# WujiangXu/AMID

Hardware: AMD Instinct MI355X
Metric: train samples/sec (higher is better)
Workload: dtype f32; 1 GPU; cloth_sport_train75-shaped SASRec train step (BASELINE.json configs[1]); batch_per_gpu=256, global_batch=256, seq_len=50, emb_dim=128, hid_dim=32, neg=1, table_rows=894820, unique_rows_last_step=1921, input=HBM-resident batch pool, dropout=on (p=0.5), optimizer=Adam (dense-equivalent lazy rows), graph=True, steps_per_graph=1, parallelism=dp1

## Files before the change

### amid_amd/csrc/adam.hip

```cpp
#include "common.h"
#include "rng.h"
#include "sort_phases.h"
#include "adam_replay.h"
#include "live_list.h"
#include "seg_spans.h"
#include "tail_parts.h"
#include "reduce_partials.h"
#include "weights_image.h"
#include "pool_slab.h"

namespace amid {

template <int MODE>
__global__ __launch_bounds__(256) void lazy_adam_rows_kernel(float* __restrict__ table, float* __restrict__ m_tab, float* __restrict__ v_tab,
                                                             int* __restrict__ last, const int* __restrict__ uniq_ids,
                                                             const int* __restrict__ n_uniq_p, const float* __restrict__ uniq_grad, int D,
                                                             const StepState* __restrict__ stp, float grad_scale) {
    __shared__ IdleCoef tab[COEF_TAB];
    const StepState st = *stp;
    const int U = *n_uniq_p;
    const int sub = threadIdx.x & 31;
    const int hw0 = blockIdx.x * (blockDim.x >> 5) + (threadIdx.x >> 5), n_hw = gridDim.x * (blockDim.x >> 5);
    if (blockIdx.x * (blockDim.x >> 5) >= U) return;
    fill_coef_table(tab, st);
// ... 356 lines not shown
        st4(g + i, gg);
        return gg;
    }
    __device__ __forceinline__ float one(long long k) const {
        float gs = reduced ? g[k] : d0[k];
        for (int r = 1; !reduced && r < world; ++r) gs += d0[r * chunk_floats + k];
        g[k] = gs;
        return gs;
    }
};

__global__ __launch_bounds__(256) void optimizer_gathered_kernel(float* __restrict__ p, float* __restrict__ m, float* __restrict__ v,
                                                                 float* __restrict__ g, long long n, int dense_blocks,
                                                                 float* __restrict__ table, float* __restrict__ m_tab, float* __restrict__ v_tab,
                                                                 int* __restrict__ last, const float* __restrict__ gathered, int world, int umax,
                                                                 long long chunk_floats, int id_rows, long long dense_off, int D, int sentinel,
                                                                 const StepState* __restrict__ stp, float grad_scale) {
    __shared__ IdleCoef tab[COEF_TAB];
    const StepState st = *stp;
    if ((int)blockIdx.x < dense_blocks) {
        dense_adam_range(p, m, v, n, blockIdx.x, dense_blocks, GatheredDenseGrad{g, gathered + dense_off, dense_off < 0, world, chunk_floats}, grad_scale,
                         adam_coef_now(st));
        return;
    }
    const int rb = blockIdx.x - dense_blocks, n_rb = gridDim.x - dense_blocks;
    const int total = world * umax;
    if (rb * 8 >= total) return;
    fill_coef_table(tab, st);
    const AdamCoef cnow = adam_coef_now(st);
    const int sub = threadIdx.x & 31;
    for (int u = rb * 8 + (threadIdx.x >> 5); u < total; u += n_rb * 8) {
        const int r0 = u / umax, i0 = u - r0 * umax;
        const int x = ((const int*)(gathered + r0 * chunk_floats))[i0];
        if (x >= sentinel) continue;
        const int half = (threadIdx.x >> 5) & 1;
        int j = -1;
        if (sub < world && sub != r0) j = find_id((const int*)(gathered + sub * chunk_floats), umax, x);
        const unsigned int fm = (unsigned int)(__ballot(j >= 0) >> (32 * half));
        if (fm & ((1u << r0) - 1u)) continue;
        const auto grad = [&](int c) {
            float4 gg = ld4(gathered + r0 * chunk_floats + (long long)(id_rows + i0) * D + 4 * c);
            for (int r = r0 + 1; r < world; ++r) {
                const int jr = __shfl(j, 32 * half + r);
                if ((fm >> r) & 1u) {
                    const float4 tt = ld4(gathered + r * chunk_floats + (long long)(id_rows + jr) * D + 4 * c);
                    gg.x += tt.x; gg.y += tt.y; gg.z += tt.z; gg.w += tt.w;
                }
            }
            return gg;
        };
        halfwave_row<ROW_STEP>(table, m_tab, v_tab, last, x, D, sub, st, tab, cnow, grad_scale, grad);
    }
}


struct DenseAdamSink {
    float* p; float* m; float* v; const float* g0; long long n; AdamCoef c; float gs;
    __device__ __forceinline__ void quad(float* dst, float4 g) const {
        const long long off = dst - g0;
        if (off < 0 || off + 4 > n) return;
        dense_quad_step(p, m, v, off, g, gs, c);
    }
    __device__ __forceinline__ void one(float* dst, float g) const {
        const long long off = dst - g0;
        if (off < 0 || off >= n) return;
        dense_elem_step(p, m, v, off, g, gs, c);
    }
};

struct DenseShipSink {
    const float* g0; long long n; float* dst;
    __device__ __forceinline__ void quad(float* d, float4 g) const {
        const long long off = d - g0;
        if (dst == nullptr || off < 0 || off + 4 > n) return;
        st4(dst + off, g);
    }
    __device__ __forceinline__ void one(float* d, float g) const {
        const long long off = d - g0;
        if (dst == nullptr || off < 0 || off >= n) return;
        dst[off] = g;
    }
};

struct TailOptArgs {
    const float* grad_rows; const int* pos_sorted; const int* seg_off; const int* seg_of; int n_sorted;
    float* uniq_grad; float* partial; int n_seg, nch; int* ticket;
    const ReduceEntry* entries; const int* blk_off; int n_entries, n_red;
    PosSum ps;
    float* p; float* m; float* v; float* g; long long n_dense; long long left_lo, left_hi; int left_blocks;
    float* table; float* m_tab; float* v_tab; int* last; const int* uniq_ids; const int* n_uniq; int row_blocks;
    const StepState* st; float grad_scale;
    float* dense_dst; int* out_ids; int n_out, pad_id, id_blocks; int* err;
};

template <int VEC, bool APPLY>
__global__ __launch_bounds__(256) void grad_tail_opt_kernel(const TailOptArgs a) {
    constexpr int D = VEC * 64;
    __shared__ IdleCoef tab[COEF_TAB];
    StepState st = {};
    if constexpr (APPLY) st = *a.st;
    const long long t = st.step;
    int bid = blockIdx.x;
    if (bid < a.n_seg) {
        segreduce_chunks_block<VEC, true>(a.grad_rows, a.pos_sorted, a.seg_of, a.n_sorted, nullptr, a.partial, bid, SEG_CHUNK, a.seg_off);
        asm volatile("s_waitcnt vmcnt(0)" ::: "memory");
        __shared__ int s_last, s_n;
        __shared__ int owners[256];
        __shared__ float red[16][D];
        __syncthreads();
        if (threadIdx.x == 0) s_last = (atomicAdd(a.ticket, 1) == a.n_seg - 1) ? 1 : 0;
        __syncthreads();
        if (!s_last) return;
        if (threadIdx.x == 0) *a.ticket = 0;
        AdamCoef cnow = {};
        if constexpr (APPLY) cnow = adam_coef_now(st);
        bool tab_filled = false;
        for (int c0 = 0; c0 < a.nch; c0 += 256) {
            if (threadIdx.x == 0) s_n = 0;
            __syncthreads();
            {
                const int c = c0 + (int)threadIdx.x;
                int u, cl;
                if (c < a.nch && spans_owner(c, a.seg_off, a.seg_of, a.n_sorted, SEG_CHUNK, u, cl) && a.seg_off[u + 1] - a.seg_off[u] > SEG_CHUNK)
                    owners[atomicAdd(&s_n, 1)] = c;
            }
            __syncthreads();
            const int n_own = s_n;
            for (int k = 0; k < n_own; ++k) {
                const int c = owners[k];
                int u = 0, c_last = 0;
                spans_owner(c, a.seg_off, a.seg_of, a.n_sorted, SEG_CHUNK, u, c_last);
                long long r = 0, l = 0;
                if constexpr (APPLY) { r = a.uniq_ids[u]; l = a.last[r]; }
                const bool lag = APPLY && row_owes(l, catchup_end(t));
                const int cq0 = threadIdx.x;
                float4 pp0 = make_float4(0.f, 0.f, 0.f, 0.f), mm0 = pp0, vv0 = pp0;
                if constexpr (APPLY) {
                    if (cq0 < D / 4) { const long long off = r * D + 4 * cq0; pp0 = ld4(a.table + off); mm0 = ld4(a.m_tab + off); vv0 = ld4(a.v_tab + off); }
                }
                spans_partials<VEC, 4, true>(red, c, c_last, a.partial);
                if (lag && !tab_filled) { fill_coef_table(tab, st); tab_filled = true; }
                __syncthreads();
                for (int cq = threadIdx.x; cq < D / 4; cq += blockDim.x) {
                    const float4 gs = make_float4(spans_total<VEC>(red, 4 * cq), spans_total<VEC>(red, 4 * cq + 1), spans_total<VEC>(red, 4 * cq + 2),
                                                  spans_total<VEC>(red, 4 * cq + 3));
                    st4(a.uniq_grad + (long long)u * D + 4 * cq, gs);
                    if constexpr (APPLY) {
                        const long long off = r * D + 4 * cq;
                        float4 pp = pp0, mm = mm0, vv = vv0;
                        row_quad_step(pp, mm, vv, gs, a.grad_scale, l, lag, st, tab, cnow);
                        st4(a.table + off, pp); st4(a.m_tab + off, mm); st4(a.v_tab + off, vv);
                    }
                }
                if constexpr (APPLY) { if (threadIdx.x == 0) a.last[r] = (int)t; }
                __syncthreads();
            }
        }
        return;
    }
    bid -= a.n_seg;
    auto make_sink = [&]() {
        if constexpr (APPLY) {
            DenseAdamSink k;
            k.p = a.p; k.m = a.m; k.v = a.v; k.g0 = a.g; k.n = a.n_dense; k.c = adam_coef_now(st); k.gs = a.grad_scale;
            return k;
        } else {
            return DenseShipSink{a.g, a.n_dense, a.dense_dst};
        }
    };
    const auto sink = make_sink();
    if (bid < a.n_red) {
        int lo = 0, hi = a.n_entries;
        while (hi - lo > 1) {
            const int mid = (lo + hi) >> 1;
            if (a.blk_off[mid] <= bid) lo = mid; else hi = mid;
        }
        reduce_partials_block(a.entries[lo], bid - a.blk_off[lo], a.blk_off[lo + 1] - a.blk_off[lo], sink);
        return;
    }
    bid -= a.n_red;
    if (bid < 2 * a.ps.nblk) {
        pos_sum_block(a.ps, D, bid / a.ps.nblk, bid % a.ps.nblk, a.ps.nblk, sink);
        return;
    }
    bid -= 2 * a.ps.nblk;
    if (bid < a.left_blocks) {
        for (long long i = a.left_lo + ((long long)bid * blockDim.x + threadIdx.x) * 4; i < a.left_hi; i += (long long)a.left_blocks * blockDim.x * 4) {
            if (i + 4 <= a.left_hi) sink.quad(a.g + i, ld4(a.g + i));
            else for (long long k = i; k < a.left_hi; ++k) sink.one(a.g + k, a.g[k]);
        }
        return;
    }
    bid -= a.left_blocks;
    if constexpr (!APPLY) {
        if (bid < a.id_blocks) {
            const int rr = bid * 256 + (int)threadIdx.x;
            if (rr < a.n_out) a.out_ids[rr] = rr < *a.n_uniq ? a.uniq_ids[rr] : a.pad_id;
            if (rr == 0 && a.err != nullptr && *a.n_uniq > a.n_out) atomicOr(a.err, AMID_FLAG_UMAX_EXCEEDED);
            return;
        }
        bid -= a.id_blocks;
    }
    {
        const int U = *a.n_uniq;
        if (bid * 8 >= U) return;
        AdamCoef cnow = {};
        if constexpr (APPLY) { fill_coef_table(tab, st); cnow = adam_coef_now(st); }
        const int sub = threadIdx.x & 31;
        for (int u = bid * 8 + (threadIdx.x >> 5); u < U; u += a.row_blocks * 8) {
            const int s0 = a.seg_off[u], s1 = a.seg_off[u + 1];
            if (s1 - s0 > SEG_CHUNK) continue;
            const int mid = min(s1, (s0 / SEG_CHUNK + 1) * SEG_CHUNK);
            const auto grad = [&](int c) {
                auto piece = [&](int e, const int e_end) {
                    float4 acc = make_float4(0.f, 0.f, 0.f, 0.f);
                    for (; e + 8 <= e_end; e += 8) {
                        int ps_[8];
#pragma unroll
                        for (int j = 0; j < 8; ++j) ps_[j] = a.pos_sorted[e + j];
                        float4 rw[8];
#pragma unroll
                        for (int j = 0; j < 8; ++j) rw[j] = ld4(a.grad_rows + (long long)ps_[j] * D + 4 * c);
#pragma unroll
                        for (int j = 0; j < 8; ++j) acc = f4add(acc, rw[j]);
                    }
                    for (; e < e_end; ++e) acc = f4add(acc, ld4(a.grad_rows + (long long)a.pos_sorted[e] * D + 4 * c));
                    return acc;
                };
                float4 gs = piece(s0, mid);
                if (mid < s1) {
                    const float4 z = make_float4(0.f, 0.f, 0.f, 0.f);
                    const float4 r0 = f4add(z, gs), r1 = f4add(z, piece(mid, s1));
                    gs = f4add(f4add(z, r0), r1);
                }
                st4(a.uniq_grad + (long long)u * D + 4 * c, gs);
                return gs;
            };
            halfwave_row<APPLY ? ROW_STEP : ROW_SHIP>(a.table, a.m_tab, a.v_tab, a.last, APPLY ? a.uniq_ids[u] : 0, D, sub, st, tab, cnow, a.grad_scale, grad);
        }
        return;
    }
}

}

using namespace amid;

extern "C" int amid_step_state_bytes(void) { return (int)sizeof(StepState); }

extern "C" int amid_step_state_pack(void* host_buf, unsigned long long seed, long long step, double lr, double beta1, double beta2, double eps) {
    AMID_CHECK_ARG(host_buf);
    StepState s;
    s.seed = seed; s.step = step; s.lr = lr; s.beta1 = beta1; s.beta2 = beta2; s.eps = eps; s.ticket = 0; s.pad_ = 0; s.step_done = step;
    *(StepState*)host_buf = s;
    return AMID_OK;
}

extern "C" int amid_step_begin(void* step_state, void* stream) {
    AMID_CHECK_ARG(step_state);
    step_begin_kernel<<<1, 1, 0, (hipStream_t)stream>>>((StepState*)step_state);
    AMID_LAUNCH_CHECK();
    return AMID_OK;
}

static inline int dense_grid(long long n, int cap) {
    long long b = (n / 4 + 255) / 256;
    if (b < 1) b = 1;
    if (b > cap) b = cap;
    return (int)b;
}

static inline int rows_grid(long long n_rows_hint) {
    long long b = (n_rows_hint + 7) / 8;
    if (b < 1) b = 1;
    if (b > 2048) b = 2048;
    return (int)b;
}

extern "C" int amid_lazy_adam_catchup_f32(float* table, float* m, float* v, int* last, const int* uniq_ids, const int* n_uniq,
                                          int n_uniq_max, int D, const void* step_state, void* stream) {
    AMID_CHECK_ARG(table && m && v && last && uniq_ids && n_uniq && step_state && D > 0 && (D % 4) == 0 && n_uniq_max > 0);
    lazy_adam_rows_kernel<0><<<rows_grid(n_uniq_max), 256, 0, (hipStream_t)stream>>>(table, m, v, last, uniq_ids, n_uniq, nullptr, D,
                                                                                      (const StepState*)step_state, 1.0f);
    AMID_LAUNCH_CHECK();
    return AMID_OK;
}

extern "C" int amid_lazy_adam_apply_f32(float* table, float* m, float* v, int* last, const int* uniq_ids, const int* n_uniq,
                                        int n_uniq_max, const float* uniq_grad, float grad_scale, int D, const void* step_state, void* stream) {
    AMID_CHECK_ARG(table && m && v && last && uniq_ids && n_uniq && uniq_grad && step_state && D > 0 && (D % 4) == 0 && n_uniq_max > 0);
    lazy_adam_rows_kernel<1><<<rows_grid(n_uniq_max), 256, 0, (hipStream_t)stream>>>(table, m, v, last, uniq_ids, n_uniq, uniq_grad, D,
                                                                                      (const StepState*)step_state, grad_scale);
    AMID_LAUNCH_CHECK();
    return AMID_OK;
}

extern "C" int amid_lazy_adam_flush_f32(float* table, float* m, float* v, int* last, long long n_rows, int D, const void* step_state,
                                        void* stream) {
    AMID_CHECK_ARG(table && m && v && last && step_state && n_rows > 0 && D > 0 && (D % 4) == 0);
    lazy_adam_flush_kernel<<<rows_grid(n_rows), 256, 0, (hipStream_t)stream>>>(table, m, v, last, n_rows, D, (const StepState*)step_state);
    AMID_LAUNCH_CHECK();
    return AMID_OK;
}

extern "C" int amid_adam_dense_f32(float* p, float* m, float* v, const float* g, long long n, float grad_scale, const void* step_state,
                                   void* stream) {
    AMID_CHECK_ARG(p && m && v && g && step_state && n > 0);
    adam_dense_kernel<<<dense_grid(n, 2048), 256, 0, (hipStream_t)stream>>>(p, m, v, g, n, (const StepState*)step_state, grad_scale);
    AMID_LAUNCH_CHECK();
    return AMID_OK;
}

static int optimizer_step(float* p, float* m, float* v, const float* g, long long n, float* table, float* m_tab, float* v_tab, int* last,
                          const int* uniq_ids, const int* n_uniq, int n_uniq_max, const float* uniq_grad, int D, float grad_scale,
                          const void* step_state, bool clip, const float* sqnorm, float max_norm, void* stream) {
    AMID_CHECK_ARG(p && m && v && g && table && m_tab && v_tab && last && uniq_ids && n_uniq && uniq_grad && step_state && D > 0 &&
                   (D % 4) == 0 && n_uniq_max > 0 && (clip ? n >= 0 && sqnorm && max_norm >= 0.0f : n > 0));
    const int db = dense_grid(n, 1024), rb = rows_grid(n_uniq_max);
    const auto kernel = clip ? optimizer_step_kernel<true> : optimizer_step_kernel<false>;
    kernel<<<db + rb, 256, 0, (hipStream_t)stream>>>(p, m, v, g, n, db, table, m_tab, v_tab, last, uniq_ids, n_uniq, uniq_grad, D,
                                                     (const StepState*)step_state, grad_scale, sqnorm, max_norm);
    AMID_LAUNCH_CHECK();
    return AMID_OK;
}

extern "C" int amid_optimizer_step_f32(float* p, float* m, float* v, const float* g, long long n, float* table, float* m_tab, float* v_tab,
                                       int* last, const int* uniq_ids, const int* n_uniq, int n_uniq_max, const float* uniq_grad, int D,
                                       float grad_scale, const void* step_state, void* stream) {
    return optimizer_step(p, m, v, g, n, table, m_tab, v_tab, last, uniq_ids, n_uniq, n_uniq_max, uniq_grad, D, grad_scale, step_state, false,
// ... 273 lines not shown
```

### amid_amd/csrc/seg_spans.h

```cpp
#pragma once
#include "common.h"

namespace amid {

constexpr int SEG_CHUNK = 64;
constexpr int SEG_CHUNK_SHORT = 16;
constexpr int SEG_BATCH = 16;

__device__ __forceinline__ int seg_of_entry(const int* __restrict__ seg_off, int U, int e) {
    int lo = 0, hi = U - 1;
    while (lo < hi) {
        const int mid = (lo + hi + 1) >> 1;
        if (seg_off[mid] <= e) lo = mid; else hi = mid - 1;
    }
    return lo;
}

template <int VEC> struct RowVec { float v[VEC]; };

template <int VEC>
__device__ __forceinline__ RowVec<VEC> load_row(const float* __restrict__ base, long long row, int D, int lane) {
    RowVec<VEC> r;
    const float* p = base + row * D + lane * VEC;
    if constexpr (VEC == 4) { float4 t = ld4(p); r.v[0] = t.x; r.v[1] = t.y; r.v[2] = t.z; r.v[3] = t.w; }
    else if constexpr (VEC == 2) { float2 t = *reinterpret_cast<const float2*>(p); r.v[0] = t.x; r.v[1] = t.y; }
    else { r.v[0] = *p; }
    return r;
}
template <int VEC>
__device__ __forceinline__ void store_row(float* __restrict__ base, long long row, int D, int lane, const RowVec<VEC>& r) {
    float* p = base + row * D + lane * VEC;
    if constexpr (VEC == 4) st4(p, make_float4(r.v[0], r.v[1], r.v[2], r.v[3]));
    else if constexpr (VEC == 2) *reinterpret_cast<float2*>(p) = make_float2(r.v[0], r.v[1]);
    else *p = r.v[0];
}

__device__ __forceinline__ bool spans_owner(int c, const int* __restrict__ seg_off, const int* __restrict__ seg_of, int n, int chunk, int& u,
                                            int& c_last) {
    const int e0 = c * chunk;
    if (e0 >= n) return false;
    const int e_end = min(e0 + chunk, n);
    if (e_end >= n) return false;
    u = seg_of[e_end - 1];
    if (seg_of[e_end] != u) return false;
    const int s_beg = seg_off[u], s_end = seg_off[u + 1];
    if (s_beg < e0) return false;
    c_last = (s_end - 1) / chunk;
    return true;
}

template <int VEC> __device__ __forceinline__ RowVec<VEC> load_row_agent(const float* __restrict__ base, long long row, int D, int lane);
template <int VEC, bool AGENT>
__device__ __forceinline__ RowVec<VEC> load_partial_row(const float* __restrict__ base, long long row, int D, int lane) {
    if constexpr (AGENT) return load_row_agent<VEC>(base, row, D, lane); else return load_row<VEC>(base, row, D, lane);
}
template <int VEC, int NW, bool AGENT = false>
__device__ __forceinline__ void spans_partials(float (*red)[VEC * 64], int c, int c_last, const float* __restrict__ partial) {
    static_assert(16 % NW == 0, "virtual waves per real wave");
    constexpr int PER = 16 / NW;
    const int D = VEC * 64;
    const int lane = lane_id(), w = wave_id();
    RowVec<VEC> acc[PER];
    int cc[PER];
#pragma unroll
    for (int j = 0; j < PER; ++j) {
        cc[j] = c + w + NW * j;
#pragma unroll
        for (int k = 0; k < VEC; ++k) acc[j].v[k] = 0.f;
    }
    constexpr int RPR = (AGENT && VEC <= 2) ? 8 : 4;
    for (bool any = true; any;) {
        any = false;
        RowVec<VEC> r[PER][RPR];
#pragma unroll
        for (int j = 0; j < PER; ++j) {
            if (cc[j] + 16 * (RPR - 1) <= c_last) {
#pragma unroll
                for (int i = 0; i < RPR; ++i) { const int ci = cc[j] + 16 * i; r[j][i] = load_partial_row<VEC, AGENT>(partial, (long long)ci * 2 + (ci == c ? 1 : 0), D, lane); }
            }
        }
#pragma unroll
        for (int j = 0; j < PER; ++j) {
            if (cc[j] + 16 * (RPR - 1) <= c_last) {
#pragma unroll
                for (int i = 0; i < RPR; ++i)
#pragma unroll
                    for (int k = 0; k < VEC; ++k) acc[j].v[k] += r[j][i].v[k];
                cc[j] += 16 * RPR;
                any = true;
            }
        }
    }
    if constexpr (RPR == 8) {
        for (bool any = true; any;) {
            any = false;
            RowVec<VEC> r[PER][4];
#pragma unroll
            for (int j = 0; j < PER; ++j) {
                if (cc[j] + 48 <= c_last) {
#pragma unroll
                    for (int i = 0; i < 4; ++i) { const int ci = cc[j] + 16 * i; r[j][i] = load_partial_row<VEC, AGENT>(partial, (long long)ci * 2 + (ci == c ? 1 : 0), D, lane); }
                }
            }
#pragma unroll
            for (int j = 0; j < PER; ++j) {
                if (cc[j] + 48 <= c_last) {
#pragma unroll
                    for (int i = 0; i < 4; ++i)
#pragma unroll
                        for (int k = 0; k < VEC; ++k) acc[j].v[k] += r[j][i].v[k];
                    cc[j] += 64;
                    any = true;
                }
            }
        }
    }
    for (bool any = true; any;) {
        any = false;
        RowVec<VEC> r[PER];
#pragma unroll
        for (int j = 0; j < PER; ++j)
            if (cc[j] <= c_last) r[j] = load_partial_row<VEC, AGENT>(partial, (long long)cc[j] * 2 + (cc[j] == c ? 1 : 0), D, lane);
#pragma unroll
        for (int j = 0; j < PER; ++j) {
            if (cc[j] <= c_last) {
#pragma unroll
                for (int k = 0; k < VEC; ++k) acc[j].v[k] += r[j].v[k];
                cc[j] += 16;
                any = true;
            }
        }
    }
#pragma unroll
    for (int j = 0; j < PER; ++j)
#pragma unroll
        for (int k = 0; k < VEC; ++k) red[w + NW * j][lane * VEC + k] = acc[j].v[k];
}
template <int VEC>
__device__ __forceinline__ float spans_total(const float (*red)[VEC * 64], int d) {
    float s = 0.f;
#pragma unroll
    for (int k = 0; k < 16; ++k) s += red[k][d];
    return s;
}

}
```

### amid_amd/engine.py

```python
from __future__ import annotations

import ctypes
import types
from dataclasses import dataclass
from typing import Dict, List, Optional, Tuple

import torch

from ._lib import lib, ptr_array

from .engine_dp import DataParallelMixin, HipMergeBackend
from .engine_graph import GraphMixin
from .engine_io import InputMixin
from .engine_topk import TopkMixin
from .plan import (DR_HEADS, SASREC_HEADS, SASREC_LN_EPS, SASREC_P_DROP, FlatParams, SasrecPlan, Shape,
                   sasrec_dense_names)

SASREC_FAMILIES = (("ln1_w", "attention_layernorms.{l}.weight"), ("ln1_b", "attention_layernorms.{l}.bias"),
                   ("w_in", "attention_layers.{l}.in_proj_weight"), ("b_in", "attention_layers.{l}.in_proj_bias"),
                   ("w_o", "attention_layers.{l}.out_proj.weight"), ("b_o", "attention_layers.{l}.out_proj.bias"),
                   ("ln2_w", "forward_layernorms.{l}.weight"), ("ln2_b", "forward_layernorms.{l}.bias"),
                   ("w1", "forward_layers.{l}.conv1.weight"), ("b1", "forward_layers.{l}.conv1.bias"),
                   ("w2", "forward_layers.{l}.conv2.weight"), ("b2", "forward_layers.{l}.conv2.bias"))
QKV_FAMILIES = tuple(n for n, _ in SASREC_FAMILIES[:4])
# ... 982 lines not shown
                L.call("amid_sas_wgrad_rows_sort_f32", ptr_array(dy), ptr_array(xx), 2, M, D, pl.splits,
                       ptr_array([pl.w_part[0].data_ptr(), pl.w_part[1].data_ptr()]), ptr_array([pl.b_part[0].data_ptr(), pl.b_part[1].data_ptr()]),
                       self._own_rows(pl), B, T, self._wgrad_mode(D), self._sort_plan_c(pl), s)
            self._enqueue_grad_tail(pl, live, seq)
            return
        L.call("amid_sas_wgrad_rows_f32", ptr_array(dy), ptr_array(xx), 2, M, D, pl.splits, ptr_array([pl.w_part[0].data_ptr(), pl.w_part[1].data_ptr()]),
               ptr_array([pl.b_part[0].data_ptr(), pl.b_part[1].data_ptr()]), self._own_rows(pl), B, T,
               self._wgrad_mode(D), s)
        if getattr(pl, "riding", False):
            L.call("amid_embed_bwd_sort_f32", (pl.dx0 if self.inc_bs else pl.dxg).data_ptr(), pl.tmq.data_ptr(), B, T, D, pl.pos_splits,
                   pl.dpos_part.data_ptr(), st, tr, SASREC_P_DROP, dom if live else None, self._sort_plan(pl), 5, s)
        elif live:
            L.call("amid_embed_bwd_rows_f32", (pl.dx0 if self.inc_bs else pl.dxg).data_ptr(), pl.tmq.data_ptr(), B, T, D, pl.pos_splits,
                   pl.dpos_part.data_ptr(), st, tr, SASREC_P_DROP, dom, s)
        else:
            L.call("amid_embed_bwd_f32", (pl.dx0 if self.inc_bs else pl.dxg).data_ptr(), pl.tmq.data_ptr(), B, T, D, pl.pos_splits,
                   pl.dpos_part.data_ptr(), st, tr, SASREC_P_DROP, s)
        if self.inc_bs:
            G = self.dense.grad
            head = (pl.dpos_part.data_ptr(), pl.pos_splits, pl.xg.data_ptr(), pl.dx0.data_ptr(), pl.inc_gate.data_ptr(), pl.inc_S.data_ptr(),
                    pl.inc_sw.data_ptr(), self._pp("inc_d{d}.trans_nn.weight"), self._pp("inc_d{d}.trans_nn.bias"),
                    self._pp("inc_d{d}.trans_bs.weight"), B, shp.T, D)
            outs = (pl.inc_dZ.data_ptr(), pl.inc_dS.data_ptr(), pl.inc_rows.data_ptr(), self._pp("inc_d{d}.trans_nn.weight", G),
                    self._pp("inc_d{d}.trans_nn.bias", G), self._pp("inc_d{d}.trans_bs.weight", G), self._pp("inc_d{d}.trans_bs.bias", G),
                    pl.dxg.data_ptr(), s)
            if getattr(pl, "inc_world", 1) > 1:
                ex = self._inc_exchange(pl)
                shard = (self.inc_bs, ex.rank * B)
                L.call("amid_inc_bwd_shard_f32", *head, *shard, 1, 1.0 / ex.world, *outs)
                self._coll(lambda: ex.all_reduce_dense(pl.inc_dZ))
                L.call("amid_inc_bwd_shard_f32", *head, *shard, 2, 1.0 / ex.world, *outs)
            else:
                L.call("amid_inc_bwd_f32", *head, *outs)
        self._enqueue_grad_tail(pl, live, seq)

    def _enqueue_grad_tail(self, pl: SasrecPlan, live: bool = False, seq: bool = False) -> None:
        L, s, shp = lib(), self.s, pl.shape
        if getattr(self, "_sort_owed", False):
            self.ev_idx.record(self.stream)
            self.enqueue_sort(pl)
        self.join_sort()
        blk = (pl.red_blk_s if seq else getattr(pl, "red_blk_v", None) if live else None) or pl.red_blk
        ent, n_ent, ent_max = ((pl.red_entries_s, pl.red_n_s, pl.red_max_s) if seq else (pl.red_entries_v, pl.red_n_v, pl.red_max_v) if live
                               else (pl.red_entries, pl.red_n, pl.red_max))
        pk = getattr(self, "_tail_pack", None)
        pl.spans_done = False
        if getattr(pl, "tail2", False) and not getattr(self, "_in_train_step", False):
            ent_t, n_ent_t, blk_t = self._tail2_table(pl)
            fp = self.dense
            head = (pl.dxg.data_ptr(), pl.pos_sorted.data_ptr(), pl.seg_off.data_ptr(), pl.seg_of.data_ptr(), pl.n_compact, self.D,
                    pl.seg_ws.data_ptr())
            mid = (ent_t.data_ptr(), n_ent_t, blk_t[0].data_ptr(), blk_t[1], pl.live.data_ptr(), shp.B, shp.Tenc,
                   fp.ptr("sac1.pos_emb.weight", fp.grad), fp.ptr("sac2.pos_emb.weight", fp.grad))
            if self.FUSED_OPT:
                left_lo = fp.slots["predictModule.fc.0.weight"][0]
                dense = (fp.grad.data_ptr(), fp.numel, left_lo, fp.numel, pl.uniq_ids.data_ptr(), pl.n_uniq.data_ptr(), pl.n_compact)
                if pk is not None:
                    from .dist import packed_rows
                    send, umax, with_dense = pk
                    id_rows, rows = packed_rows(umax, self.D)
                    L.call("amid_grad_tail_live_dp1_f32", *head, send.data_ptr() + 4 * id_rows * self.D, *mid, *dense, umax, self.n_rows,
                           send.data_ptr(), send.data_ptr() + 4 * rows * self.D if with_dense else None, pl.err.data_ptr(),
                           pl.tail_ticket.data_ptr(), s)
                else:
                    L.call("amid_grad_tail_live_dp1_f32", *head, pl.uniq_grad.data_ptr(), *mid, *dense, 0, 0, None, None, None,
                           pl.tail_ticket.data_ptr(), s)
            elif pk is not None:
                from .dist import packed_rows
                send, umax, with_dense = pk
                id_rows, rows = packed_rows(umax, self.D)
                L.call("amid_grad_tail_live_dp_f32", *head, send.data_ptr() + 4 * id_rows * self.D, *mid, pl.uniq_ids.data_ptr(),
                       pl.n_uniq.data_ptr(), umax, self.n_rows, send.data_ptr(), self.dense.grad.data_ptr() if with_dense else None,
                       send.data_ptr() + 4 * rows * self.D if with_dense else None, self.dense.numel if with_dense else 0,
                       pl.err.data_ptr(), s)
            else:
                L.call("amid_grad_tail_live_dp_f32", *head, pl.uniq_grad.data_ptr(), *mid, None, None, 0, 0, None, None, None, 0, None, s)
            pl.spans_done = True
            return
        pl.opt_done = False
        if getattr(pl, "tail2", False) and self.FUSED_OPT and self.table_m is not None and not self.dr:
            ent_t, n_ent_t, blk_t = self._tail2_table(pl)
            fp = self.dense
            left_lo = fp.slots["predictModule.fc.0.weight"][0]
            L.call("amid_grad_tail_opt_f32", pl.dxg.data_ptr(), pl.pos_sorted.data_ptr(), pl.seg_off.data_ptr(), pl.seg_of.data_ptr(), pl.n_compact,
                   self.D, pl.seg_ws.data_ptr(), pl.uniq_grad.data_ptr(), ent_t.data_ptr(), n_ent_t, blk_t[0].data_ptr(), blk_t[1],
                   pl.live.data_ptr(), shp.B, shp.Tenc, fp.ptr("sac1.pos_emb.weight", fp.grad), fp.ptr("sac2.pos_emb.weight", fp.grad),
                   fp.data.data_ptr(), fp.m.data_ptr(), fp.v.data_ptr(), fp.grad.data_ptr(), fp.numel, left_lo, fp.numel,
                   self.table.data_ptr(), self.table_m.data_ptr(), self.table_v.data_ptr(), self.table_last.data_ptr(), pl.uniq_ids.data_ptr(),
                   pl.n_uniq.data_ptr(), pl.n_compact, self.grad_scale, self.step_state.data_ptr(), pl.tail_ticket.data_ptr(), s)
            pl.opt_done = True
            return
        if getattr(pl, "tail2", False):
            ent_t, n_ent_t, blk_t = self._tail2_table(pl)
            fp = self.dense
            L.call("amid_grad_tail_live_f32", pl.dxg.data_ptr(), pl.pos_sorted.data_ptr(), pl.seg_off.data_ptr(), pl.seg_of.data_ptr(), pl.n_compact,
                   self.D, pl.seg_ws.data_ptr(), pl.uniq_grad.data_ptr(), ent_t.data_ptr(), n_ent_t, blk_t[0].data_ptr(), blk_t[1],
                   pl.live.data_ptr(), shp.B, shp.Tenc, fp.ptr("sac1.pos_emb.weight", fp.grad), fp.ptr("sac2.pos_emb.weight", fp.grad),
                   None, None, None, 0, 0, None, None, None, None, s)
            return
        if pk is not None:
            from .dist import packed_rows
            send, umax, with_dense = pk
            id_rows, rows = packed_rows(umax, self.D)
            L.call("amid_grad_tail_pack_f32", pl.dxg.data_ptr(), pl.pos_sorted.data_ptr(), pl.seg_off.data_ptr(), pl.seg_of.data_ptr(), self.n_sparse(pl),
                   self.D, pl.seg_ws.data_ptr(), send.data_ptr() + 4 * id_rows * self.D, ent.data_ptr(),
                   n_ent, ent_max, pl.uniq_ids.data_ptr(), pl.n_uniq.data_ptr(), umax,
                   self.n_rows, send.data_ptr(), self.dense.grad.data_ptr() if with_dense else None,
                   send.data_ptr() + 4 * rows * self.D if with_dense else None, self.dense.numel if with_dense else 0,
                   pl.err.data_ptr(), blk[0].data_ptr(), blk[1], s)
            return
        spans_later = bool(self.FUSED_SPANS and getattr(self, "_in_train_step", False) and self.D in (64, 128, 256))
        left = getattr(pl, "red_left_s" if seq else "red_left_v" if (live and hasattr(pl, "red_left_v")) else "red_left", None)
        if spans_later and self.FUSED_OPT and self.table_m is not None and left is not None:
            fp = self.dense
            L.call("amid_grad_tail_opt_f32", pl.dxg.data_ptr(), pl.pos_sorted.data_ptr(), pl.seg_off.data_ptr(), pl.seg_of.data_ptr(), self.n_sparse(pl),
                   self.D, pl.seg_ws.data_ptr(), pl.uniq_grad.data_ptr(), ent.data_ptr(), n_ent, blk[0].data_ptr(), blk[1],
                   None, 0, 0, None, None, fp.data.data_ptr(), fp.m.data_ptr(), fp.v.data_ptr(), fp.grad.data_ptr(), fp.numel, *(left or (0, 0)),
                   self.table.data_ptr(), self.table_m.data_ptr(), self.table_v.data_ptr(), self.table_last.data_ptr(), pl.uniq_ids.data_ptr(),
                   pl.n_uniq.data_ptr(), self.n_sparse(pl), self.grad_scale, self.step_state.data_ptr(), pl.tail_ticket.data_ptr(), s)
            pl.opt_done = True
            return
        pl.spans_owed = self.n_sparse(pl) if spans_later else 0
        L.call("amid_grad_tail_nospans_f32" if spans_later else "amid_grad_tail_f32", pl.dxg.data_ptr(), pl.pos_sorted.data_ptr(), pl.seg_off.data_ptr(),
               pl.seg_of.data_ptr(), self.n_sparse(pl), self.D, pl.seg_ws.data_ptr(), pl.uniq_grad.data_ptr(), ent.data_ptr(), n_ent, ent_max,
               blk[0].data_ptr(), blk[1], s)

    def enqueue_optimizer(self, pl: SasrecPlan, sparse=None) -> None:
        L, s = lib(), self.s
        self._ensure_opt_state()
        fp = self.dense
        if sparse is None:
            ids, rows, nu, cap = pl.uniq_ids, pl.uniq_grad, pl.n_uniq, self.n_sparse(pl)
        else:
            ids, rows, nu = sparse
            cap = ids.numel()
        if getattr(pl, "opt_done", False):
            pl.opt_done = False
            if sparse is not None:
                raise RuntimeError("the gradient tail already applied this step's local gradients")
            return
        owed = int(getattr(pl, "spans_owed", 0))
        pl.spans_owed = 0
        t2 = getattr(pl, "tail2", False) and not getattr(pl, "spans_done", False)
        if sparse is None and (t2 or owed):
            L.call("amid_optimizer_step_spans_f32", fp.data.data_ptr(), fp.m.data_ptr(), fp.v.data_ptr(), fp.grad.data_ptr(), fp.numel,
                   self.table.data_ptr(), self.table_m.data_ptr(), self.table_v.data_ptr(), self.table_last.data_ptr(), ids.data_ptr(),
                   nu.data_ptr(), cap, rows.data_ptr(), self.D, self.grad_scale, self.step_state.data_ptr(), pl.seg_off.data_ptr(),
                   pl.seg_of.data_ptr(), pl.n_compact if t2 else owed, pl.seg_ws.data_ptr(), s)
            return
        if owed:
            raise RuntimeError("the gradient tail left the chunk-crossing runs to an optimizer launch that takes merged lists")
        L.call("amid_optimizer_step_f32", fp.data.data_ptr(), fp.m.data_ptr(), fp.v.data_ptr(), fp.grad.data_ptr(), fp.numel,
               self.table.data_ptr(), self.table_m.data_ptr(), self.table_v.data_ptr(), self.table_last.data_ptr(), ids.data_ptr(),
               nu.data_ptr(), cap, rows.data_ptr(), self.D, self.grad_scale, self.step_state.data_ptr(), s)

    def enqueue_loop_optimizer(self, pl: SasrecPlan, g: torch.Tensor, sqnorm: Optional[torch.Tensor] = None, max_norm: float = float("inf")) -> None:
        self._ensure_opt_state()
        if getattr(pl, "opt_done", False) or int(getattr(pl, "spans_owed", 0)):
            raise RuntimeError("the plan's last backward was a fused train step's: its gradients are applied already")
        fp = self.dense
        args = (fp.data.data_ptr(), fp.m.data_ptr(), fp.v.data_ptr(), g.data_ptr(), fp.numel, self.table.data_ptr(), self.table_m.data_ptr(),
                self.table_v.data_ptr(), self.table_last.data_ptr(), pl.uniq_ids.data_ptr(), pl.n_uniq.data_ptr(), self.n_sparse(pl),
                pl.uniq_grad.data_ptr(), self.D, self.grad_scale, self.step_state.data_ptr())
        if sqnorm is None:
            lib().call("amid_optimizer_step_f32", *args, self.s)
        else:
            lib().call("amid_optimizer_step_clip_f32", *args, sqnorm.data_ptr(), float(max_norm), self.s)

    def enqueue_grad_sqnorm(self, pl: SasrecPlan, g: torch.Tensor, out: torch.Tensor) -> None:
        ws = getattr(self, "_sqnorm_ws", None)
        if ws is None:
            ws = self._sqnorm_ws = torch.empty(lib().value("amid_grad_sqnorm_workspace_bytes"), dtype=torch.uint8, device=self.device)
# ... 380 lines not shown
```

### amid_amd/engine_io.py

```python
from __future__ import annotations

import ctypes
import os
from dataclasses import dataclass
from typing import Dict, List, Optional, Tuple

import torch

from ._lib import lib, ptr_array

from .plan import SasrecPlan


class InputMixin:
    def load_batch(self, pl: SasrecPlan, i_node, neg_samples, seq_d1, seq_d2, labels=None, domain_id=None, ob_label=None) -> None:
        if self.input_pool(pl) is not None:
            raise RuntimeError("this plan reads its batches from an installed input pool (set_input_pool); drop the pool before loading single batches")
        with torch.cuda.stream(self.stream):
            pl.in_i_node.copy_(i_node.reshape(-1), non_blocking=True)
            pl.in_neg.copy_(neg_samples.reshape(pl.shape.B, -1), non_blocking=True)
            pl.in_seq_d1.copy_(seq_d1, non_blocking=True)
            pl.in_seq_d2.copy_(seq_d2, non_blocking=True)
            if labels is not None:
                pl.labels.copy_(labels.reshape(pl.shape.B, -1), non_blocking=True)
                pl.domain.copy_(domain_id.reshape(-1), non_blocking=True)
            if ob_label is not None:
                pl.in_ob.copy_(ob_label.reshape(-1), non_blocking=True)

    def pack_batch(self, pl: SasrecPlan, i_node, neg_samples, seq_d1, seq_d2, labels, domain_id) -> torch.Tensor:
        B, NI = pl.shape.B, pl.shape.NI
        lab = torch.zeros(2 * ((B * NI + 1) // 2), dtype=torch.float32, device=labels.device)
        lab[: B * NI] = labels.reshape(-1).float()
        return torch.cat((i_node.reshape(-1).long(), neg_samples.reshape(-1).long(), seq_d1.reshape(-1).long(), seq_d2.reshape(-1).long(),
                          domain_id.reshape(-1).long(), lab.view(torch.int64))).contiguous()

    def pack_epoch(self, pl: SasrecPlan, i_node, neg_samples, seq_d1, seq_d2, labels, domain_id, ob_label=None) -> torch.Tensor:
        B, NI = pl.shape.B, pl.shape.NI
        n = i_node.shape[0]
        lab = torch.zeros(2 * ((B * NI + 1) // 2), dtype=torch.float32, device=i_node.device)
        lab[: B * NI] = labels.reshape(-1).float()
        parts = [i_node.reshape(n, -1).long(), neg_samples.reshape(n, -1).long(), seq_d1.reshape(n, -1).long(), seq_d2.reshape(n, -1).long(),
                 domain_id.reshape(n, -1).long(), lab.view(torch.int64).unsqueeze(0).expand(n, -1)]
        if pl.in_ob is not None:
            parts.append((ob_label if ob_label is not None else torch.zeros_like(domain_id)).reshape(n, -1).long())
        out = torch.cat(parts, 1).contiguous()
        if out.shape[1] != pl.in_words:
            raise ValueError(f"packed row has {out.shape[1]} words, the plan expects {pl.in_words}")
        return out

    def set_input_pool(self, pl: SasrecPlan, pool: Optional[torch.Tensor]) -> None:
        key = self._graph_key()
        if pool is not None:
            if pool.dtype != torch.int64 or pool.dim() != 2 or pool.shape[1] != pl.in_words or pool.stride(1) != 1 \
                    or pool.device != pl.in_pack.device:
                raise ValueError(f"input pool must be a device int64 [n, {pl.in_words}] tensor with contiguous rows")
            pl.pools[key] = [pool, (-self.step) % pool.shape[0]]
            self._prepare_pool(pl, key, pool, alloc=True)
        else:
            pl.pools.pop(key, None)
            getattr(pl, "slabs", {}).pop(key, None)
        torch.cuda.synchronize(self.device)
        if getattr(pl, "graphs", None):
            pl.graphs.pop(key, None)
        if getattr(pl, "graphs_n", None):
            for k in [k for k in pl.graphs_n if k[0] == key]:
                pl.graphs_n.pop(k)
        if getattr(pl, "dp_graphs", None):
            pl.dp_graphs.clear()
        pl.graphs_local = {}

    def input_pool(self, pl: SasrecPlan):
        return pl.pools.get(self._graph_key()) if getattr(pl, "pools", None) else None

    def refill_input_pool(self, pl: SasrecPlan, pool: torch.Tensor) -> bool:
        ent = self.input_pool(pl)
        if ent is None or ent[0].shape != pool.shape or (-self.step) % pool.shape[0] != ent[1]:
            return False
        with torch.cuda.stream(self.stream):
            ent[0].copy_(pool, non_blocking=True)
        self._prepare_pool(pl, self._graph_key(), ent[0], alloc=False)
        return True

    def _prepared_pool_ok(self, pl: SasrecPlan, n_pool: int) -> bool:
        if not getattr(self, "PREPARED_POOL", False) or not hasattr(self, "_tail2_ok") or getattr(self, "compute", "") == "bf16":
            return False
        shp = pl.shape
        if lib().value("amid_pool_prepare_workspace_bytes", n_pool, shp.B, shp.T, shp.NI - 1, self.n_rows) <= 0:
            return False
        saved = getattr(self, "_in_train_step", False)
        self._in_train_step = True
        try:
            return bool(self._tail2_ok(pl))
        finally:
            self._in_train_step = saved

    def _prepare_pool(self, pl: SasrecPlan, key, pool: torch.Tensor, alloc: bool) -> None:
        if not hasattr(pl, "slabs"):
            pl.slabs = {}
        L, shp, n_pool = lib(), pl.shape, pool.shape[0]
        if alloc:
            pl.slabs.pop(key, None)
            if not self._prepared_pool_ok(pl, n_pool):
                return
            ints = L.value("amid_pool_slab_ints", shp.B, shp.T, shp.NI - 1)
            slab = torch.zeros(n_pool, ints, dtype=torch.int32, device=pool.device)
            ws = torch.empty(L.value("amid_pool_prepare_workspace_bytes", n_pool, shp.B, shp.T, shp.NI - 1, self.n_rows), dtype=torch.uint8,
                             device=pool.device)
            pl.slabs[key] = (slab, ws)
            torch.cuda.synchronize(self.device)
        ent = pl.slabs.get(key)
        if ent is None:
            return
        slab, ws = ent
        L.call("amid_pool_prepare_i32", pool.data_ptr(), pool.stride(0), n_pool, pl.in_words, shp.B, shp.T, shp.NI - 1, self.n_rows,
               slab.data_ptr(), slab.stride(0), ws.data_ptr(), self.s)

    def pool_slabs(self, pl: SasrecPlan):
        return pl.slabs.get(self._graph_key()) if getattr(pl, "slabs", None) else None

    def load_packed(self, pl: SasrecPlan, packed: torch.Tensor) -> None:
        if self.input_pool(pl) is not None:
            raise RuntimeError("this plan reads its batches from an installed input pool (set_input_pool); drop the pool before loading single batches")
        with torch.cuda.stream(self.stream):
            pl.in_pack.copy_(packed, non_blocking=True)
```

Measured before the change: 908,400 samples/s.

## Reorder grad tail blocks, cache span owners, and size row grid by pool unique max

The fused grad-tail kernel now places per-row reduce+Adam blocks right after the segment-chunk blocks instead of last. Row blocks prefetch positions, table/m/v rows via shuffle-broadcast indices, and fill the coefficient table only when some row lags. The last-ticket block records owner metadata in shared memory so span ownership is not recomputed. The span-partials loader issues all loads before accumulating. Host code launches row blocks sized to the maximum unique count seen across the prepared pool rather than n_compact, which trims idle blocks but relies on that precomputed bound. Optional timestamp instrumentation is compiled out by default.

Result: no change. 911,900 samples/s (median of 2 runs) (+0.4%).

```diff
diff --git a/amid_amd/csrc/adam.hip b/amid_amd/csrc/adam.hip
--- a/amid_amd/csrc/adam.hip
+++ b/amid_amd/csrc/adam.hip
@@ -462,6 +462,30 @@
     }
 };
 
+enum TailRole { TAIL_CHUNK, TAIL_LAST_TICKET, TAIL_ROWS, TAIL_ROWS_IDLE, TAIL_SUMS, TAIL_POS, TAIL_LEFT, TAIL_IDS };
+#ifdef AMID_TAIL_STAMPS
+constexpr int TAIL_STAMP_BLOCKS = 4096;
+static __device__ unsigned long long amid_tail_stamp_buf[TAIL_STAMP_BLOCKS * 4 * 2];
+static __device__ int amid_tail_stamp_role[TAIL_STAMP_BLOCKS];
+static __device__ unsigned long long amid_tail_stamp_last[32];
+struct TailStamp {
+    int role = TAIL_CHUNK;
+    __device__ __forceinline__ TailStamp() {
+        if (lane_id() == 0 && blockIdx.x < TAIL_STAMP_BLOCKS) amid_tail_stamp_buf[(blockIdx.x * 4 + wave_id()) * 2] = __builtin_amdgcn_s_memrealtime();
+    }
+    __device__ __forceinline__ ~TailStamp() {
+        if (lane_id() == 0 && blockIdx.x < TAIL_STAMP_BLOCKS) amid_tail_stamp_buf[(blockIdx.x * 4 + wave_id()) * 2 + 1] = __builtin_amdgcn_s_memrealtime();
+        if (threadIdx.x == 0 && blockIdx.x < TAIL_STAMP_BLOCKS) amid_tail_stamp_role[blockIdx.x] = role;
+    }
+};
+#define TAIL_MOMENT(i) do { if (threadIdx.x == 0 && (i) < 32) amid_tail_stamp_last[i] = __builtin_amdgcn_s_memrealtime(); } while (0)
+#define TAIL_NOTE(i, v) do { if (threadIdx.x == 0 && (i) < 32) amid_tail_stamp_last[i] = (unsigned long long)(v); } while (0)
+#else
+struct TailStamp { int role; };
+#define TAIL_MOMENT(i) do { } while (0)
+#define TAIL_NOTE(i, v) do { } while (0)
+#endif
+
 struct TailOptArgs {
     const float* grad_rows; const int* pos_sorted; const int* seg_off; const int* seg_of; int n_sorted;
     float* uniq_grad; float* partial; int n_seg, nch; int* ticket;
@@ -476,6 +500,7 @@
 template <int VEC, bool APPLY>
 __global__ __launch_bounds__(256) void grad_tail_opt_kernel(const TailOptArgs a) {
     constexpr int D = VEC * 64;
+    TailStamp ts;
     __shared__ IdleCoef tab[COEF_TAB];
     StepState st = {};
     if constexpr (APPLY) st = *a.st;
@@ -486,11 +511,14 @@
         asm volatile("s_waitcnt vmcnt(0)" ::: "memory");
         __shared__ int s_last, s_n;
         __shared__ int owners[256];
+        __shared__ int own_u[256], own_last[256], own_row[256], own_stamp[256];
         __shared__ float red[16][D];
         __syncthreads();
         if (threadIdx.x == 0) s_last = (atomicAdd(a.ticket, 1) == a.n_seg - 1) ? 1 : 0;
         __syncthreads();
         if (!s_last) return;
+        ts.role = TAIL_LAST_TICKET;
+        TAIL_MOMENT(0);
         if (threadIdx.x == 0) *a.ticket = 0;
         AdamCoef cnow = {};
         if constexpr (APPLY) cnow = adam_coef_now(st);
@@ -500,27 +528,41 @@
             __syncthreads();
             {
                 const int c = c0 + (int)threadIdx.x;
-                int u, cl;
-                if (c < a.nch && spans_owner(c, a.seg_off, a.seg_of, a.n_sorted, SEG_CHUNK, u, cl) && a.seg_off[u + 1] - a.seg_off[u] > SEG_CHUNK)
-                    owners[atomicAdd(&s_n, 1)] = c;
+                const int e0 = c * SEG_CHUNK, e_end = min(e0 + SEG_CHUNK, a.n_sorted);
+                if (c < a.nch && e_end < a.n_sorted) {
+                    const int u = a.seg_of[e_end - 1];
+                    if (a.seg_of[e_end] == u) {
+                        const int s_beg = a.seg_off[u], s_end = a.seg_off[u + 1];
+                        int r = 0;
+                        if constexpr (APPLY) r = a.uniq_ids[u];
+                        if (s_beg >= e0 && s_end - s_beg > SEG_CHUNK) {
+                            const int k = atomicAdd(&s_n, 1);
+                            owners[k] = c; own_u[k] = u; own_last[k] = (s_end - 1) / SEG_CHUNK;
+                            if constexpr (APPLY) { own_row[k] = r; own_stamp[k] = a.last[r]; }
+                        }
+                    }
+                }
             }
             __syncthreads();
             const int n_own = s_n;
+            if (c0 == 0) { TAIL_MOMENT(1); TAIL_NOTE(2, n_own); }
             for (int k = 0; k < n_own; ++k) {
                 const int c = owners[k];
-                int u = 0, c_last = 0;
-                spans_owner(c, a.seg_off, a.seg_of, a.n_sorted, SEG_CHUNK, u, c_last);
+                const int u = own_u[k], c_last = own_last[k];
                 long long r = 0, l = 0;
-                if constexpr (APPLY) { r = a.uniq_ids[u]; l = a.last[r]; }
+                if constexpr (APPLY) { r = own_row[k]; l = own_stamp[k]; }
                 const bool lag = APPLY && row_owes(l, catchup_end(t));
                 const int cq0 = threadIdx.x;
                 float4 pp0 = make_float4(0.f, 0.f, 0.f, 0.f), mm0 = pp0, vv0 = pp0;
                 if constexpr (APPLY) {
                     if (cq0 < D / 4) { const long long off = r * D + 4 * cq0; pp0 = ld4(a.table + off); mm0 = ld4(a.m_tab + off); vv0 = ld4(a.v_tab + off); }
                 }
+                TAIL_MOMENT(4 + 4 * k);
+                TAIL_NOTE(7 + 4 * k, c_last - c + 1);
                 spans_partials<VEC, 4, true>(red, c, c_last, a.partial);
                 if (lag && !tab_filled) { fill_coef_table(tab, st); tab_filled = true; }
                 __syncthreads();
+                TAIL_MOMENT(5 + 4 * k);
                 for (int cq = threadIdx.x; cq < D / 4; cq += blockDim.x) {
                     const float4 gs = make_float4(spans_total<VEC>(red, 4 * cq), spans_total<VEC>(red, 4 * cq + 1), spans_total<VEC>(red, 4 * cq + 2),
                                                   spans_total<VEC>(red, 4 * cq + 3));
@@ -533,12 +575,101 @@
                     }
                 }
                 if constexpr (APPLY) { if (threadIdx.x == 0) a.last[r] = (int)t; }
+                TAIL_MOMENT(6 + 4 * k);
                 __syncthreads();
             }
         }
         return;
     }
     bid -= a.n_seg;
+    if (bid < a.row_blocks) {
+        const int U = *a.n_uniq;
+        ts.role = TAIL_ROWS_IDLE;
+        if (bid * 8 >= U) return;
+        ts.role = TAIL_ROWS;
+        const int sub = threadIdx.x & 31, stride = a.row_blocks * 8, u_first = bid * 8 + (threadIdx.x >> 5);
+        const long long end = catchup_end(t);
+        struct RowIn { int s0, s1, pa, pb; long long r, l; float4 p, m, v; };
+        const auto request = [&](int u) {
+            RowIn in = {};
+            in.s0 = a.seg_off[u]; in.s1 = a.seg_off[u + 1];
+            if constexpr (APPLY) in.r = a.uniq_ids[u];
+            if (in.s1 - in.s0 > SEG_CHUNK) return in;
+            if constexpr (APPLY) {
+                in.l = a.last[in.r];
+                if (sub < D / 4) { const long long off = in.r * D + 4 * sub; in.p = ld4(a.table + off); in.m = ld4(a.m_tab + off); in.v = ld4(a.v_tab + off); }
+            }
+            if (in.s0 + sub < in.s1) in.pa = a.pos_sorted[in.s0 + sub];
+            if (in.s0 + 32 + sub < in.s1) in.pb = a.pos_sorted[in.s0 + 32 + sub];
+            return in;
+        };
+        RowIn in = {};
+        bool lag_mine = false;
+        if (u_first < U) {
+            in = request(u_first);
+            if constexpr (APPLY) {
+                lag_mine = row_owes(in.l, end);
+                for (int u = u_first + stride; u < U; u += stride) lag_mine = lag_mine || row_owes(a.last[a.uniq_ids[u]], end);
+            }
+        }
+        AdamCoef cnow = {};
+        if constexpr (APPLY) {
+            if (__syncthreads_or(lag_mine ? 1 : 0)) fill_coef_table(tab, st);
+            cnow = adam_coef_now(st);
+        }
+        for (int u = u_first; u < U; u += stride) {
+            if (u != u_first) in = request(u);
+            const int n = in.s1 - in.s0;
+            if (n > SEG_CHUNK) continue;
+            const int nmid = min(in.s1, (in.s0 / SEG_CHUNK + 1) * SEG_CHUNK) - in.s0;
+            const bool lag = APPLY && row_owes(in.l, end);
+            for (int c0 = 0; c0 < D / 4; c0 += 32) {
+                const int c = c0 + sub;
+                const bool act = c < D / 4;
+                float4 p = in.p, m = in.m, v = in.v;
+                if constexpr (APPLY) {
+                    if (c0 > 0 && act) { const long long off = in.r * D + 4 * c; p = ld4(a.table + off); m = ld4(a.m_tab + off); v = ld4(a.v_tab + off); }
+                }
+                const auto piece = [&](int j, const int j_end) {
+                    float4 acc = make_float4(0.f, 0.f, 0.f, 0.f);
+                    for (; j < j_end; j += 8) {
+                        float4 rw[8];
+#pragma unroll
+                        for (int k = 0; k < 8; ++k) {
+                            const int jj = j + k;
+                            if (jj < j_end) {
+                                const int ps = __shfl(jj < 32 ? in.pa : in.pb, jj & 31, 32);
+                                if (act) rw[k] = ld4(a.grad_rows + (long long)ps * D + 4 * c);
+                            }
+                        }
+#pragma unroll
+                        for (int k = 0; k < 8; ++k) if (j + k < j_end) acc = f4add(acc, rw[k]);
+                    }
+                    return acc;
+                };
+                float4 gs = piece(0, nmid);
+                if (nmid < n) {
+                    const float4 z = make_float4(0.f, 0.f, 0.f, 0.f);
+                    const float4 r0 = f4add(z, gs), r1 = f4add(z, piece(nmid, n));
+                    gs = f4add(f4add(z, r0), r1);
+                }
+                if (act) {
+                    st4(a.uniq_grad + (long long)u * D + 4 * c, gs);
+                    if constexpr (APPLY) {
+                        const long long off = in.r * D + 4 * c;
+                        row_quad_step(p, m, v, gs, a.grad_scale, in.l, lag, st, tab, cnow);
+                        st4(a.table + off, p); st4(a.m_tab + off, m); st4(a.v_tab + off, v);
+                    }
+                }
+            }
+            if constexpr (APPLY) {
+                __builtin_amdgcn_wave_barrier();
+                if (sub == 0) a.last[in.r] = (int)t;
+            }
+        }
+        return;
+    }
+    bid -= a.row_blocks;
     auto make_sink = [&]() {
         if constexpr (APPLY) {
             DenseAdamSink k;
@@ -550,6 +681,7 @@
     };
     const auto sink = make_sink();
     if (bid < a.n_red) {
+        ts.role = TAIL_SUMS;
         int lo = 0, hi = a.n_entries;
         while (hi - lo > 1) {
             const int mid = (lo + hi) >> 1;
@@ -560,11 +692,13 @@
     }
     bid -= a.n_red;
     if (bid < 2 * a.ps.nblk) {
+        ts.role = TAIL_POS;
         pos_sum_block(a.ps, D, bid / a.ps.nblk, bid % a.ps.nblk, a.ps.nblk, sink);
         return;
     }
     bid -= 2 * a.ps.nblk;
     if (bid < a.left_blocks) {
+        ts.role = TAIL_LEFT;
         for (long long i = a.left_lo + ((long long)bid * blockDim.x + threadIdx.x) * 4; i < a.left_hi; i += (long long)a.left_blocks * blockDim.x * 4) {
             if (i + 4 <= a.left_hi) sink.quad(a.g + i, ld4(a.g + i));
             else for (long long k = i; k < a.left_hi; ++k) sink.one(a.g + k, a.g[k]);
@@ -574,6 +708,7 @@
     bid -= a.left_blocks;
     if constexpr (!APPLY) {
         if (bid < a.id_blocks) {
+            ts.role = TAIL_IDS;
             const int rr = bid * 256 + (int)threadIdx.x;
             if (rr < a.n_out) a.out_ids[rr] = rr < *a.n_uniq ? a.uniq_ids[rr] : a.pad_id;
             if (rr == 0 && a.err != nullptr && *a.n_uniq > a.n_out) atomicOr(a.err, AMID_FLAG_UMAX_EXCEEDED);
@@ -581,50 +716,22 @@
         }
         bid -= a.id_blocks;
     }
-    {
-        const int U = *a.n_uniq;
-        if (bid * 8 >= U) return;
-        AdamCoef cnow = {};
-        if constexpr (APPLY) { fill_coef_table(tab, st); cnow = adam_coef_now(st); }
-        const int sub = threadIdx.x & 31;
-        for (int u = bid * 8 + (threadIdx.x >> 5); u < U; u += a.row_blocks * 8) {
-            const int s0 = a.seg_off[u], s1 = a.seg_off[u + 1];
-            if (s1 - s0 > SEG_CHUNK) continue;
-            const int mid = min(s1, (s0 / SEG_CHUNK + 1) * SEG_CHUNK);
-            const auto grad = [&](int c) {
-                auto piece = [&](int e, const int e_end) {
-                    float4 acc = make_float4(0.f, 0.f, 0.f, 0.f);
-                    for (; e + 8 <= e_end; e += 8) {
-                        int ps_[8];
-#pragma unroll
-                        for (int j = 0; j < 8; ++j) ps_[j] = a.pos_sorted[e + j];
-                        float4 rw[8];
-#pragma unroll
-                        for (int j = 0; j < 8; ++j) rw[j] = ld4(a.grad_rows + (long long)ps_[j] * D + 4 * c);
-#pragma unroll
-                        for (int j = 0; j < 8; ++j) acc = f4add(acc, rw[j]);
-                    }
-                    for (; e < e_end; ++e) acc = f4add(acc, ld4(a.grad_rows + (long long)a.pos_sorted[e] * D + 4 * c));
-                    return acc;
-                };
-                float4 gs = piece(s0, mid);
-                if (mid < s1) {
-                    const float4 z = make_float4(0.f, 0.f, 0.f, 0.f);
-                    const float4 r0 = f4add(z, gs), r1 = f4add(z, piece(mid, s1));
-                    gs = f4add(f4add(z, r0), r1);
-                }
-                st4(a.uniq_grad + (long long)u * D + 4 * c, gs);
-                return gs;
-            };
-            halfwave_row<APPLY ? ROW_STEP : ROW_SHIP>(a.table, a.m_tab, a.v_tab, a.last, APPLY ? a.uniq_ids[u] : 0, D, sub, st, tab, cnow, a.grad_scale, grad);
-        }
-        return;
-    }
 }
 
 }
 
 using namespace amid;
+
+#ifdef AMID_TAIL_STAMPS
+extern "C" int amid_tail_stamps_read(unsigned long long* host) {
+    constexpr int NW = TAIL_STAMP_BLOCKS * 8;
+    if (int e = (int)hipMemcpyFromSymbol(host, HIP_SYMBOL(amid::amid_tail_stamp_buf), sizeof(unsigned long long) * NW)) return e;
+    static int roles[TAIL_STAMP_BLOCKS];
+    if (int e = (int)hipMemcpyFromSymbol(roles, HIP_SYMBOL(amid::amid_tail_stamp_role), sizeof(roles))) return e;
+    for (int i = 0; i < TAIL_STAMP_BLOCKS; ++i) host[NW + i] = (unsigned long long)roles[i];
+    return (int)hipMemcpyFromSymbol(host + NW + TAIL_STAMP_BLOCKS, HIP_SYMBOL(amid::amid_tail_stamp_last), sizeof(unsigned long long) * 32);
+}
+#endif
 
 extern "C" int amid_step_state_bytes(void) { return (int)sizeof(StepState); }
 
diff --git a/amid_amd/csrc/seg_spans.h b/amid_amd/csrc/seg_spans.h
--- a/amid_amd/csrc/seg_spans.h
+++ b/amid_amd/csrc/seg_spans.h
@@ -91,6 +91,29 @@
             }
         }
     }
+    if constexpr (AGENT) {
+        RowVec<VEC> r[PER][RPR - 1];
+#pragma unroll
+        for (int j = 0; j < PER; ++j)
+#pragma unroll
+            for (int i = 0; i < RPR - 1; ++i) {
+                const int ci = min(cc[j] + 16 * i, c_last);
+                r[j][i] = load_partial_row<VEC, AGENT>(partial, (long long)ci * 2 + (ci == c ? 1 : 0), D, lane);
+            }
+#pragma unroll
+        for (int j = 0; j < PER; ++j)
+#pragma unroll
+            for (int i = 0; i < RPR - 1; ++i)
+                if (cc[j] + 16 * i <= c_last) {
+#pragma unroll
+                    for (int k = 0; k < VEC; ++k) acc[j].v[k] += r[j][i].v[k];
+                }
+#pragma unroll
+        for (int j = 0; j < PER; ++j)
+#pragma unroll
+            for (int k = 0; k < VEC; ++k) red[w + NW * j][lane * VEC + k] = acc[j].v[k];
+        return;
+    }
     if constexpr (RPR == 8) {
         for (bool any = true; any;) {
             any = false;
diff --git a/amid_amd/engine.py b/amid_amd/engine.py
--- a/amid_amd/engine.py
+++ b/amid_amd/engine.py
@@ -1088,12 +1088,14 @@
             ent_t, n_ent_t, blk_t = self._tail2_table(pl)
             fp = self.dense
             left_lo = fp.slots["predictModule.fc.0.weight"][0]
+            umax = getattr(pl, "slab_umax", {}).get(self._graph_key()) if getattr(pl, "prepared", False) else None
+            n_uniq_max = min(pl.n_compact, max(umax, 1)) if umax is not None else pl.n_compact
             L.call("amid_grad_tail_opt_f32", pl.dxg.data_ptr(), pl.pos_sorted.data_ptr(), pl.seg_off.data_ptr(), pl.seg_of.data_ptr(), pl.n_compact,
                    self.D, pl.seg_ws.data_ptr(), pl.uniq_grad.data_ptr(), ent_t.data_ptr(), n_ent_t, blk_t[0].data_ptr(), blk_t[1],
                    pl.live.data_ptr(), shp.B, shp.Tenc, fp.ptr("sac1.pos_emb.weight", fp.grad), fp.ptr("sac2.pos_emb.weight", fp.grad),
                    fp.data.data_ptr(), fp.m.data_ptr(), fp.v.data_ptr(), fp.grad.data_ptr(), fp.numel, left_lo, fp.numel,
                    self.table.data_ptr(), self.table_m.data_ptr(), self.table_v.data_ptr(), self.table_last.data_ptr(), pl.uniq_ids.data_ptr(),
-                   pl.n_uniq.data_ptr(), pl.n_compact, self.grad_scale, self.step_state.data_ptr(), pl.tail_ticket.data_ptr(), s)
+                   pl.n_uniq.data_ptr(), n_uniq_max, self.grad_scale, self.step_state.data_ptr(), pl.tail_ticket.data_ptr(), s)
             pl.opt_done = True
             return
         if getattr(pl, "tail2", False):
diff --git a/amid_amd/engine_io.py b/amid_amd/engine_io.py
--- a/amid_amd/engine_io.py
+++ b/amid_amd/engine_io.py
@@ -59,6 +59,7 @@
         else:
             pl.pools.pop(key, None)
             getattr(pl, "slabs", {}).pop(key, None)
+            getattr(pl, "slab_umax", {}).pop(key, None)
         torch.cuda.synchronize(self.device)
         if getattr(pl, "graphs", None):
             pl.graphs.pop(key, None)
@@ -100,6 +101,7 @@
         L, shp, n_pool = lib(), pl.shape, pool.shape[0]
         if alloc:
             pl.slabs.pop(key, None)
+            getattr(pl, "slab_umax", {}).pop(key, None)
             if not self._prepared_pool_ok(pl, n_pool):
                 return
             ints = L.value("amid_pool_slab_ints", shp.B, shp.T, shp.NI - 1)
@@ -114,6 +116,11 @@
         slab, ws = ent
         L.call("amid_pool_prepare_i32", pool.data_ptr(), pool.stride(0), n_pool, pl.in_words, shp.B, shp.T, shp.NI - 1, self.n_rows,
                slab.data_ptr(), slab.stride(0), ws.data_ptr(), self.s)
+        if alloc:
+            self.sync()
+            if not hasattr(pl, "slab_umax"):
+                pl.slab_umax = {}
+            pl.slab_umax[key] = int(slab[:, 0].max().item())
 
     def pool_slabs(self, pl: SasrecPlan):
         return pl.slabs.get(self._graph_key()) if getattr(pl, "slabs", None) else None
```
